# hari-krishnan/openglottal

Measured on AMD Instinct MI355X. Metric: frames/sec 256×256 U-Net-only (frames resident in HBM), higher is better.
Workload: dtype f32; 1 GPU; U-Net-only 256x256 grayscale synthetic video (BASELINE configs[1]; configs[3] with --total-frames 10000), features (32,64,128,256), frames = RandomState(1234+i) BGR -> gray, frame loop u8->/255->UNet->sigmoid->>0.5->area, gray frames resident in HBM, int32 areas left on the device; frames_this_rank=512, frames_per_launch=64, hip_graphs=True, lanes=2

## Files before the change

openglottal_amd/csrc/og_kernels.hpp:

```cpp
#pragma once
#include <hip/hip_runtime.h>
#include <stdint.h>

typedef float f32x16 __attribute__((ext_vector_type(16)));
typedef float f32x4 __attribute__((ext_vector_type(4)));

#define OG_GLOBAL_AS __attribute__((address_space(1)))
#define OG_LDS_AS __attribute__((address_space(3)))

__device__ __forceinline__ void glds16(const float* gsrc, unsigned lds_wave_base) {
    unsigned keep;
    asm volatile(
        "s_mov_b32 %0, m0\n\t"
        "s_mov_b32 m0, %2\n\t"
        "s_nop 0\n\t"
        "global_load_lds_dwordx4 %1, off\n\t"
        "s_mov_b32 m0, %0"
        : "=&s"(keep)
        : "v"(gsrc), "s"(lds_wave_base)
        : "memory");
}
typedef float f32x2 __attribute__((ext_vector_type(2)));
__device__ __forceinline__ f32x2 og_fma2s(f32x2 a, f32x2 b, f32x2 c) { return f32x2{fmaf(a.x, b.x, c.x), fmaf(a.y, b.y, c.y)}; }
__device__ __forceinline__ f32x2 og_fma2(f32x2 a, f32x2 b, f32x2 c) { return __builtin_elementwise_fma(a, b, c); }
// ... 922 lines not shown
    for (int c = c_lo; c < c_hi; ++c) {
#pragma unroll
        for (int t = 0; t < TAPS; ++t) {
            if (VS && ((MODE == 3) ? (t == 0 && c == vnext) : (c * TAPS_ + t == vnext))) {
#pragma unroll
                for (int m = 0; m < MS; ++m) {
#pragma unroll
                    for (int r = 0; r < 16; ++r) {
                        vsum[m][r] += acc[m][r];
                        acc[m][r] = 0.f;
                    }
                }
                ++vp;
                vnext = (vp < vs_n) ? __builtin_amdgcn_readfirstlane((vp * vs_units) / vs_n) : -1;
            }
            if (MODE == 0 && ks_n > 1 && (c * TAPS + t < s_lo || c * TAPS + t >= s_hi)) continue;
            if (MODE == 3) {
                const int par = c / cpc;
                if (((t >> 1) == 0 && (par & 2) == 0) || ((t & 1) == 0 && (par & 1) == 0)) continue;
            }
            const int stg = (NSTG == 3) ? t % 3 : (step & 1), stg_next = (NSTG == 3) ? (t + 1) % 3 : ((step + 1) & 1);
            if (step + 1 < step_end) stage_w(stg_next, step + 1);

            const unsigned wb = (unsigned)stg * WBYTES;
            const int dy = (MODE == 0) ? t / 3 : (MODE == 3) ? (t >> 1) : 0;
            const int dx = (MODE == 0) ? t % 3 : (MODE == 3) ? (t & 1) : 0;
#pragma unroll
            for (int j = 0; j < 4; ++j) {
                const f32x4 bv = og_lds_read16(bbase[j] + wb);
#pragma unroll
                for (int m = 0; m < MS; ++m) {
                    const f32x4 av = og_lds_read16(abase[dx][j ^ ((dy & 1) << 1)] + (unsigned)((dy + 2 * m) * (HW_ * 128)));
                    acc[m] = __builtin_amdgcn_mfma_f32_32x32x2f32(av.x, bv.x, acc[m], 0, 0, 0);
                    acc[m] = __builtin_amdgcn_mfma_f32_32x32x2f32(av.y, bv.y, acc[m], 0, 0, 0);
                    acc[m] = __builtin_amdgcn_mfma_f32_32x32x2f32(av.z, bv.z, acc[m], 0, 0, 0);
                    acc[m] = __builtin_amdgcn_mfma_f32_32x32x2f32(av.w, bv.w, acc[m], 0, 0, 0);
                }
            }
            og_wait_dma();
            __syncthreads();
            ++step;
        }
        if (c + 1 < c_hi) {
            stage_halo(c + 1);
            og_wait_dma();
            __syncthreads();
        }
    }

    if (st != nullptr && tid == 0) st[2] = __builtin_amdgcn_s_memtime();
    if (a.prio_mode == 3) __builtin_amdgcn_s_setprio(3);
    if (VS && vs_n > 1) {
#pragma unroll
        for (int m = 0; m < MS; ++m)
#pragma unroll
            for (int r = 0; r < 16; ++r) acc[m][r] = vsum[m][r] + acc[m][r];
    }
    if (ks_n > 1) {
        float* pw = a.partial + ((long long)item_id * 4 + wave) * (MS * 16 * 64) + lane;
        if (a.tile_counter == nullptr) {
#pragma unroll
            for (int m = 0; m < MS; ++m)
#pragma unroll
                for (int r = 0; r < 16; ++r) pw[(m * 16 + r) * 64] = acc[m][r];
        } else {
#pragma unroll
            for (int m = 0; m < MS; ++m)
#pragma unroll
                for (int r = 0; r < 16; ++r) __hip_atomic_store(pw + (m * 16 + r) * 64, acc[m][r], __ATOMIC_RELAXED, __HIP_MEMORY_SCOPE_AGENT);
        }
        if (a.tile_counter != nullptr) {
            asm volatile("s_waitcnt vmcnt(0)" ::: "memory");
            __syncthreads();
            int* const flag = (int*)smem;
            if (tid == 0) *flag = (atomicAdd(a.tile_counter + tile_id, 1) == ks_n - 1) ? 1 : 0;
            __syncthreads();
            if (*(volatile int*)flag) {
#pragma unroll
                for (int m = 0; m < MS; ++m)
#pragma unroll
                    for (int r = 0; r < 16; ++r) acc[m][r] = 0.f;
                constexpr int PG = (MS == 1) ? 4 : (MS == 2) ? 2 : 1;
                for (int sp_ = 0; sp_ < ks_n; sp_ += PG) {
                    float pv[PG][MS * 16];
#pragma unroll
                    for (int g = 0; g < PG; ++g) {
                        const int sg = (sp_ + g < ks_n) ? sp_ + g : sp_;
                        const float* pr = a.partial + (((long long)tile_id * ks_n + sg) * 4 + wave) * (MS * 16 * 64) + lane;
#pragma unroll
                        for (int k = 0; k < MS * 16; ++k) pv[g][k] = __hip_atomic_load(pr + k * 64, __ATOMIC_RELAXED, __HIP_MEMORY_SCOPE_AGENT);
                    }
#pragma unroll
                    for (int g = 0; g < PG; ++g)
                        if (sp_ + g < ks_n) {
#pragma unroll
                            for (int m = 0; m < MS; ++m)
#pragma unroll
                                for (int r = 0; r < 16; ++r) acc[m][r] += pv[g][m * 16 + r];
                        }
                }
                __syncthreads();
                unsigned char* const scr = smem + wave * 5120;
                if (a.act == 1) conv_epilogue_b<NT, MODE, TH, 1, false>(a, acc, n_tile, b, ty0, tx0, wm, wn, li, lh, esc, esh, scr);
                else if (a.act == 2 && a.res != nullptr) conv_epilogue_b<NT, MODE, TH, 2, true>(a, acc, n_tile, b, ty0, tx0, wm, wn, li, lh, esc, esh, scr);
                else if (a.act == 2) conv_epilogue_b<NT, MODE, TH, 2, false>(a, acc, n_tile, b, ty0, tx0, wm, wn, li, lh, esc, esh, scr);
                else conv_epilogue_b<NT, MODE, TH, 0, false>(a, acc, n_tile, b, ty0, tx0, wm, wn, li, lh, esc, esh, scr);
                if (tid == 0) a.tile_counter[tile_id] = 0;
            }
        }
    } else {
        unsigned char* const scr = smem + wave * 5120;
        if (a.act == 1) conv_epilogue_b<NT, MODE, TH, 1, false>(a, acc, n_tile, b, ty0, tx0, wm, wn, li, lh, esc, esh, scr);
        else if (a.act == 2 && a.res != nullptr) conv_epilogue_b<NT, MODE, TH, 2, true>(a, acc, n_tile, b, ty0, tx0, wm, wn, li, lh, esc, esh, scr);
        else if (a.act == 2) conv_epilogue_b<NT, MODE, TH, 2, false>(a, acc, n_tile, b, ty0, tx0, wm, wn, li, lh, esc, esh, scr);
        else conv_epilogue_b<NT, MODE, TH, 0, false>(a, acc, n_tile, b, ty0, tx0, wm, wn, li, lh, esc, esh, scr);
    }
    if (st != nullptr && tid == 0) {
        asm volatile("s_waitcnt vmcnt(0)" ::: "memory");
        st[3] = __builtin_amdgcn_s_memtime();
    }
}

__device__ __forceinline__ f32x2 og_add2(f32x2 a, f32x2 b) {
    f32x2 r;
    asm volatile("v_pk_add_f32 %0, %1, %2" : "=v"(r) : "v"(a), "v"(b));
    return r;
}
__device__ __forceinline__ f32x2 og_sub2(f32x2 a, f32x2 b) {
    f32x2 r;
    asm volatile("v_pk_add_f32 %0, %1, %2 neg_lo:[0,1] neg_hi:[0,1]" : "=v"(r) : "v"(a), "v"(b));
    return r;
}

template <int NT, int ACT, bool POOL, int HEAD>
__device__ __forceinline__ void wino_tile_end(const ConvArgs& a, const f32x2 (&p)[2][4][4], int n_tile, int b, int ty0, int tx0, int wm, int wn,
                                              int li, int lh, float sc, float sh, unsigned char* scratch) {
    static_assert(NT == 1 || HEAD == 0, "the fused head sits on a 32-column layer");
    constexpr int AREA = 1280;
    const int lane = li + 32 * lh;
    const int cbase = n_tile * 32 * NT + wn * 32;
    const int W = a.W;
    const int ys = ty0 + 8 * wm;
    const int rrow = lane >> 3, rc4 = (lane & 7) * 4;
    const int xl = 2 * (rrow >> 2) + (rrow & 1), yl = (rrow & 3) >> 1;

    const __amdgpu_buffer_rsrc_t out_rs = og_rsrc(a.out + (long long)b * a.out_frame_stride, (unsigned)a.out_frame_stride * 4u);
    unsigned vq[4];
#pragma unroll
    for (int q = 0; q < 4; ++q)
        vq[q] = (tx0 + xl + 4 * q < W) ? (unsigned)(((yl * W + xl + 4 * q) * a.out_pix_stride + rc4) * 4) : OG_OOB;
    unsigned so = (unsigned)(((ys * W + tx0) * a.out_pix_stride + a.out_ch_off + cbase) * 4);
    const unsigned so_step = (unsigned)(2 * W * a.out_pix_stride * 4);

    float* const fw = (float*)scratch + (128 * lh + li);
    const float* const fr = (const float*)scratch + rrow * 32 + rc4;
    __amdgpu_buffer_rsrc_t pool_rs = out_rs;
    unsigned vpool = 0, pso = 0, pso_step = 0;
    if (POOL) {
        pool_rs = og_rsrc(a.pool + (long long)b * a.pool_frame_stride, (unsigned)a.pool_frame_stride * 4u);
        vpool = (tx0 + 2 * rrow < W) ? (unsigned)((rrow * a.pool_pix_stride + rc4) * 4) : OG_OOB;
        pso = (unsigned)((((ys >> 1) * (W >> 1) + (tx0 >> 1)) * a.pool_pix_stride + a.pool_ch_off + cbase) * 4);
        pso_step = (unsigned)((W >> 1) * a.pool_pix_stride * 4);
    }
    f32x4 wv = {0.f, 0.f, 0.f, 0.f};
    int hbx1 = 0, hby1 = 0, hbx2 = 1 << 30, hby2 = 1 << 30, head_cnt = 0;
    const int hk = lane & 7;
    unsigned vh = OG_OOB;
    unsigned hso = 0;
    __amdgpu_buffer_rsrc_t lrs = out_rs, mrs = out_rs;
    if (HEAD) {
        wv = *(const f32x4*)(a.head_w + rc4);
        if (a.head_boxes != nullptr) {
            hbx1 = a.head_boxes[b * 4 + 0];
            hby1 = a.head_boxes[b * 4 + 1];
            hbx2 = a.head_boxes[b * 4 + 2];
            hby2 = a.head_boxes[b * 4 + 3];
            if (hbx1 < 0) { hbx1 = hby1 = hbx2 = hby2 = 0; }
        }
        if (hk < 4 && tx0 + xl + 4 * hk < W) vh = (unsigned)(yl * W + xl + 4 * hk);
        hso = (unsigned)(ys * W + tx0);
        const unsigned long long hfo = (unsigned long long)((long long)b * a.H * W);
        lrs = og_rsrc((const void*)((unsigned long long)a.head_logits + hfo * 4ull), a.head_logits ? (unsigned)(a.H * W) * 4u : 0u);
        mrs = og_rsrc((const void*)((unsigned long long)a.head_mask + hfo), a.head_mask ? (unsigned)(a.H * W) : 0u);
    }

    const f32x2 sc2 = {sc, sc}, sh2 = {sh, sh};
#pragma unroll
    for (int mp = 0; mp < 2; ++mp) {
        f32x2 vmaxs[4];
#pragma unroll
        for (int g = 0; g < 4; ++g) {
#pragma unroll
            for (int rr = 0; rr < 4; ++rr) {
                f32x2 v = og_fma2(p[mp][g][rr], sc2, sh2);
                if (ACT == 1) v = f32x2{fmaxf(v.x, 0.f), fmaxf(v.y, 0.f)};
                fw[(8 * g + rr) * 32] = v.x;
                fw[AREA + (8 * g + rr) * 32] = v.y;
                if (POOL) vmaxs[g] = (rr == 0) ? v : f32x2{fmaxf(vmaxs[g].x, v.x), fmaxf(vmaxs[g].y, v.y)};
            }
        }
        if (POOL) {
#pragma unroll
            for (int g = 0; g < 4; ++g) {
                fw[1024 - 96 * lh + g * 64] = vmaxs[g].x;
                fw[AREA + 1024 - 96 * lh + g * 64] = vmaxs[g].y;
            }
        }
        f32x4 v4[2][4], p4[2];
#pragma unroll
        for (int s = 0; s < 2; ++s) {
#pragma unroll
            for (int q = 0; q < 4; ++q) v4[s][q] = *(const f32x4*)(fr + s * AREA + q * 256);
            if (POOL) p4[s] = *(const f32x4*)(fr + s * AREA + 1024);
        }
#pragma unroll
        for (int s = 0; s < 2; ++s) {
            if (HEAD != 1) {
#pragma unroll
                for (int q = 0; q < 4; ++q) og_buffer_store16(v4[s][q], out_rs, vq[q], so);
                so += so_step;
            }
            if (HEAD) {
                float sd[4];
#pragma unroll
                for (int q = 0; q < 4; ++q) {
                    float sdot = 0.f;
                    sdot = fmaf(v4[s][q].x, wv.x, sdot);
                    sdot = fmaf(v4[s][q].y, wv.y, sdot);
                    sdot = fmaf(v4[s][q].z, wv.z, sdot);
                    sdot = fmaf(v4[s][q].w, wv.w, sdot);
                    sdot += __shfl_xor(sdot, 1);
                    sdot += __shfl_xor(sdot, 2);
                    sdot += __shfl_xor(sdot, 4);
                    sd[q] = sdot;
                }
                float mine = sd[3];
                mine = (hk == 2) ? sd[2] : mine;
                mine = (hk == 1) ? sd[1] : mine;
                mine = (hk == 0) ? sd[0] : mine;
                const float lg = mine + a.head_bias;
                const float prob = 1.0f / (1.0f + expf(-lg));
                const bool on = prob > a.head_thr;
                const int x = tx0 + xl + 4 * hk, y = ys + 2 * (2 * mp + s) + yl;
                const bool counted = on && vh != OG_OOB && x >= hbx1 && x < hbx2 && y >= hby1 && y < hby2;
                head_cnt += __builtin_popcountll(__ballot(counted));
                __builtin_amdgcn_raw_buffer_store_b32(__builtin_bit_cast(unsigned, lg), lrs, (vh == OG_OOB) ? OG_OOB : vh * 4u, hso * 4u, 0);
                __builtin_amdgcn_raw_buffer_store_b8((unsigned char)(on ? 255 : 0), mrs, vh, hso, 0);
                hso += 2u * (unsigned)W;
            }
            if (POOL) {
                og_buffer_store16(p4[s], pool_rs, vpool, pso);
                pso += pso_step;
            }
        }
    }
    if (HEAD && a.head_area != nullptr) {
        if (lane == 0) {
            const int tile = (ty0 / 32) * a.tiles_x + (tx0 >> 4);
            a.head_area[((long long)b * a.tiles_x * a.tiles_y + tile) * 4 + wm] = head_cnt;
        }
    }
}

template <int NT>
__global__ __launch_bounds__(256, 1) void k_conv_wino(ConvArgs a) {
    constexpr int KC = 8 * NT;
    constexpr int PB = KC * 4;
    constexpr int SL = KC / 4;
    constexpr int KS = KC / 8;
    constexpr int TH = 32 / NT;
    constexpr int RP = 18;
    constexpr int RAW_PIX = (TH + 2) * RP;
    constexpr int RAW_BYTES = RAW_PIX * PB;
    constexpr int V_BYTES = 16 * 4096;
    constexpr int UP_BYTES = 32 * NT * PB;
    constexpr int UG_BYTES = 8 * UP_BYTES;
    constexpr int U_IT = UG_BYTES / 4096;
    constexpr int RAW_PIECES = RAW_PIX * SL;
    constexpr int RAW_IT = (RAW_PIECES + 255) / 256;
    constexpr int NST = 8 * KS;

    extern __shared__ __attribute__((aligned(16))) unsigned char smem[];
    const int tid = threadIdx.x;
    const int lane = tid & 63;
    const int wave = __builtin_amdgcn_readfirstlane(tid >> 6);
    const int wn = (NT == 2) ? (wave & 1) : 0, wm = (NT == 2) ? (wave >> 1) : wave;
    const int li = lane & 31, lh = lane >> 5;

    int n_tile, b;
    og_zdecode(a, (int)blockIdx.z, n_tile, b);
    if (b >= a.frames) return;
    const int ty0 = (int)blockIdx.y * TH, tx0 = (int)blockIdx.x * 16;
    unsigned long long* st = nullptr;
    if (a.stamps != nullptr) {
        const unsigned wg = og_wg_index();
        st = a.stamps + 8ull * (wg < 511u ? wg : 511u);
        if (tid == 0) st[0] = __builtin_amdgcn_s_memtime();
    }

    const og_i32x4 in_rsrc = og_make_rsrc(a.in + (long long)b * a.in_frame_stride + a.in_ch_off,
                                          (unsigned)(a.in_frame_stride - a.in_ch_off) * 4u);
    unsigned hoff[RAW_IT];
    {
        constexpr int QY = (256 / SL) / RP, QR = (256 / SL) % RP;
        const int pc = tid % SL;
        int hy = (tid / SL) / RP, r = (tid / SL) - hy * RP;
#pragma unroll
        for (int it = 0; it < RAW_IT; ++it) {
            const int hx = (r >= 9) ? 2 * (r - 9) + 1 : 2 * r;
            const int gy = ty0 + hy - 1, gx = tx0 + hx - 1;
            const bool inb = it * 256 + tid < RAW_PIECES && (unsigned)gy < (unsigned)a.H && (unsigned)gx < (unsigned)a.W;
            hoff[it] = inb ? (unsigned)((gy * a.W + gx) * a.in_pix_stride * 4 + pc * 16) : OG_OOB;
            hy += QY;
            r += QR;
            if (r >= RP) { r -= RP; hy += 1; }
        }
    }
    const unsigned long long last_mask = __builtin_amdgcn_ballot_w64(((RAW_IT - 1) * 256 + tid) < RAW_PIECES);
    const unsigned lds0 = og_lds_addr(smem);
    const int n_ck = a.n_chunks * (32 / KC);
    const og_i32x4 w_rsrc = og_make_rsrc(a.wpk + (long long)n_tile * n_ck * (16 * UP_BYTES / 4), (unsigned)n_ck * (16u * UP_BYTES));
    const unsigned woff = (unsigned)tid * 16u;
    const unsigned ubase = __builtin_amdgcn_readfirstlane(lds0 + RAW_BYTES + V_BYTES + wave * 1024);
    const unsigned hbase = __builtin_amdgcn_readfirstlane(lds0 + wave * 1024);
    unsigned wso = 0, hso = 0;
    auto u_piece = [&](auto pad_, int stage, int i) {
        glds16b_m0<decltype(pad_)::value != 0>(woff, w_rsrc, wso + i * 4096, ubase + stage * UG_BYTES + i * 4096);
    };
    auto raw_piece = [&](auto pad_, int it) {
        if (it < RAW_IT - 1) glds16b_m0<decltype(pad_)::value != 0>(hoff[it], in_rsrc, hso, hbase + it * 4096);
        else glds16b_m0_masked(hoff[it], in_rsrc, hso, hbase + it * 4096, last_mask);
    };
#pragma unroll
    for (int it = 0; it < RAW_IT; ++it) raw_piece(og_const<1>{}, it);
#pragma unroll
    for (int i = 0; i < U_IT; ++i) u_piece(og_const<1>{}, 0, i);
    wso = UG_BYTES;
    hso = PB;
    if (st != nullptr && tid == 0) st[1] = __builtin_amdgcn_s_memtime();

    const int wxa = 2 * (li >> 3) + ((li >> 2) & 1);
    const int nb = wn * 32 + li;
    unsigned abase[KS], bbase[KS];
#pragma unroll
    for (int j = 0; j < KS; ++j) {
        if (NT == 2) {
            abase[j] = lds0 + RAW_BYTES + ((4 * wm + (li & 3)) * 8 + wxa) * 64 + (((2 * j + lh) ^ (li & 3)) << 4);
            bbase[j] = lds0 + RAW_BYTES + V_BYTES + nb * 64 + (((2 * j + lh) ^ ((nb >> 2) & 3)) << 4);
        } else {
            abase[j] = lds0 + RAW_BYTES + (8 * (4 * wm + (wxa >> 1)) + (li & 3) + 4 * (wxa & 1)) * 32 + ((lh ^ ((wxa >> 1) & 1)) << 4);
            bbase[j] = lds0 + RAW_BYTES + V_BYTES + nb * 32 + ((lh ^ ((nb >> 3) & 1)) << 4);
        }
        asm volatile("" : "+v"(abase[j]));
        asm volatile("" : "+v"(bbase[j]));
    }
    const int qc = tid % SL;
    const int wr = (NT == 2) ? (tid >> 5) : 4 * (tid >> 6) + ((tid >> 1) & 3);
    const int wc = (NT == 2) ? ((tid >> 2) & 7) : ((tid >> 3) & 1) + 2 * ((tid >> 4) & 3);
    const int wt = 8 * wr + wc;
    unsigned rbase = lds0 + (unsigned)((2 * wr * RP + wc) * PB + qc * 16);
    unsigned vwbase = (NT == 2) ? lds0 + RAW_BYTES + (unsigned)(wt * 64 + ((qc ^ (wr & 3)) << 4))
                                : lds0 + RAW_BYTES + (unsigned)((8 * (4 * (wr >> 2) + (wc >> 1)) + (wr & 3) + 4 * (wc & 1)) * 32 + ((qc ^ ((wc >> 1) & 1)) << 4));
    asm volatile("" : "+v"(rbase));
    asm volatile("" : "+v"(vwbase));

    const int ecol = n_tile * 32 * NT + wn * 32 + li;
    const float esc = a.scale[ecol], esh = a.shift[ecol];

    f32x16 acc[16];
#pragma unroll
    for (int k = 0; k < 16; ++k) {
#pragma unroll
        for (int r = 0; r < 16; ++r) acc[k][r] = 0.f;
        asm volatile("" : "+a"(acc[k]));
    }

    f32x4 d[16], t[16], tv[16];
    auto raw_read = [&](int n) {
        const int i = n >> 2, j = n & 3;
        d[n] = og_lds_read16(rbase + (unsigned)((i * RP + (j & 1) * 9 + (j >> 1)) * PB));
    };
    auto row_op = [&](int n) {
        const int r = n >> 2, j = n & 3;
        t[n] = (r == 0) ? og_sub4(d[0 + j], d[8 + j]) : (r == 1) ? og_add4(d[4 + j], d[8 + j]) : (r == 2) ? og_sub4(d[8 + j], d[4 + j]) : og_sub4(d[4 + j], d[12 + j]);
    };
    auto col_op = [&](int n) {
        const int i = n >> 2, cc = n & 3;
        tv[n] = (cc == 0) ? og_sub4(t[4 * i + 0], t[4 * i + 2]) : (cc == 1) ? og_add4(t[4 * i + 1], t[4 * i + 2]) : (cc == 2) ? og_sub4(t[4 * i + 2], t[4 * i + 1])
                                                                                                                     : og_sub4(t[4 * i + 1], t[4 * i + 3]);
    };
    auto v_write = [&](int k) { *(OG_LDS_AS f32x4*)(unsigned long long)(vwbase + (unsigned)(k * 4096)) = tv[k]; };
    auto xf_op = [&](int n) {
        if (n < 16) raw_read(n);
        else if (n < 32) row_op(n - 16);
        else if (n < 48) col_op(n - 32);
        else if (n < 56) v_write(n - 48);
    };
    auto xf4 = [&](int n) { xf_op(n); xf_op(n + 1); xf_op(n + 2); xf_op(n + 3); };

    og_wait_dma();
    if (st != nullptr && tid == 0) st[2] = __builtin_amdgcn_s_memtime();
    __syncthreads();
#pragma unroll
    for (int n = 0; n < 48; ++n) xf_op(n);
#pragma unroll
    for (int k = 0; k < 8; ++k) v_write(k);
    __syncthreads();
    if (st != nullptr && tid == 0) st[3] = __builtin_amdgcn_s_memtime();

    auto group = [&](auto g_, auto nxt_) {
        constexpr int g = decltype(g_)::value;
        constexpr bool NXT = decltype(nxt_)::value != 0;
        constexpr bool MORE_U = (g == 0) || NXT;
        f32x4 fa[2], fb[2];
        fa[0] = og_lds_read16(abase[0] + (unsigned)(8 * g * 4096));
        fb[0] = og_lds_read16(bbase[0] + (unsigned)(g * UG_BYTES));
#pragma unroll
        for (int st = 0; st < NST; ++st) {
            const int k = 8 * g + st / KS;
            const f32x4 av = fa[st & 1], bv = fb[st & 1];
            acc[k] = __builtin_amdgcn_mfma_f32_32x32x2f32(av.x, bv.x, acc[k], 0, 0, 0);
            __builtin_amdgcn_sched_barrier(0);
            if (st + 1 < NST) {
                const int kn = (st + 1) / KS, jn = (st + 1) % KS;
                fa[(st + 1) & 1] = og_lds_read16(abase[jn] + (unsigned)((8 * g + kn) * 4096));
                fb[(st + 1) & 1] = og_lds_read16(bbase[jn] + (unsigned)(g * UG_BYTES + kn * UP_BYTES));
            }
            __builtin_amdgcn_sched_barrier(0);
            acc[k] = __builtin_amdgcn_mfma_f32_32x32x2f32(av.y, bv.y, acc[k], 0, 0, 0);
            __builtin_amdgcn_sched_barrier(0);
            if constexpr (g == 0) {
                if (NT == 2) { if (st < 8) v_write(8 + st); }
                else v_write(8 + st);
            } else if constexpr (NXT) {
                if (NT == 2) {
                    if (st < 2) xf4(8 * st);
                    else if (st >= 3 && st < 7) { xf_op(16 + 4 * (st - 3)); xf_op(16 + 4 * (st - 3) + 1); }
                    else if (st >= 7 && st < 11) { xf_op(32 + 4 * (st - 7)); xf_op(32 + 4 * (st - 7) + 1); }
                    else if (st >= 11 && st < 15) xf_op(48 + 2 * (st - 11));
                } else {
                    if (st < 2) xf4(8 * st);
                    else if (st < 4) xf4(16 + 8 * (st - 2));
                    else if (st < 6) xf4(32 + 8 * (st - 4));
                    else { xf_op(48 + 4 * (st - 6)); xf_op(48 + 4 * (st - 6) + 1); }
                }
            }
            __builtin_amdgcn_sched_barrier(0);
            acc[k] = __builtin_amdgcn_mfma_f32_32x32x2f32(av.z, bv.z, acc[k], 0, 0, 0);
            __builtin_amdgcn_sched_barrier(0);
            if constexpr (MORE_U) {
                if (st < U_IT) u_piece(og_const<0>{}, g ^ 1, st);
            }
            if constexpr (g == 1 && NXT) {
                if (NT == 2) {
                    if (st < 2) xf4(8 * st + 4);
                    else if (st >= 3 && st < 7) { xf_op(16 + 4 * (st - 3) + 2); xf_op(16 + 4 * (st - 3) + 3); }
                    else if (st >= 7 && st < 11) { xf_op(32 + 4 * (st - 7) + 2); xf_op(32 + 4 * (st - 7) + 3); }
                    else if (st >= 11 && st < 15) xf_op(48 + 2 * (st - 11) + 1);
                } else {
                    if (st < 2) xf4(8 * st + 4);
                    else if (st < 4) xf4(16 + 8 * (st - 2) + 4);
                    else if (st < 6) xf4(32 + 8 * (st - 4) + 4);
                    else { xf_op(48 + 4 * (st - 6) + 2); xf_op(48 + 4 * (st - 6) + 3); }
                }
            }
            __builtin_amdgcn_sched_barrier(0);
            acc[k] = __builtin_amdgcn_mfma_f32_32x32x2f32(av.w, bv.w, acc[k], 0, 0, 0);
            __builtin_amdgcn_sched_barrier(0);
            if constexpr (g == 0 && NXT) {
                if (st < RAW_IT) raw_piece(og_const<0>{}, st);
            }
            __builtin_amdgcn_sched_barrier(0);
        }
        wso += UG_BYTES;
        if constexpr (g == 0) hso += PB;
        og_wait_dma();
        __syncthreads();
    };
    for (int c = 0; c < n_ck - 1; ++c) {
        group(og_const<0>{}, og_const<1>{});
        group(og_const<1>{}, og_const<1>{});
    }
    group(og_const<0>{}, og_const<0>{});
    group(og_const<1>{}, og_const<0>{});

    if (st != nullptr && tid == 0) st[4] = __builtin_amdgcn_s_memtime();
    f32x2 o[2][4][4];
#pragma unroll
    for (int mp = 0; mp < 2; ++mp) {
#pragma unroll
        for (int g = 0; g < 4; ++g) {
            const int r = 4 * g + 2 * mp;
#pragma unroll
            for (int k = 0; k < 16; ++k) asm volatile("" : "+a"(acc[k]));
            f32x2 tm[2][4];
#pragma unroll
            for (int j = 0; j < 4; ++j) {
                const f32x2 m0 = {acc[0 + j][r], acc[0 + j][r + 1]}, m1 = {acc[4 + j][r], acc[4 + j][r + 1]};
                const f32x2 m2 = {acc[8 + j][r], acc[8 + j][r + 1]}, m3 = {acc[12 + j][r], acc[12 + j][r + 1]};
                tm[0][j] = og_add2(og_add2(m0, m1), m2);
                tm[1][j] = og_sub2(og_sub2(m1, m2), m3);
            }
#pragma unroll
            for (int y = 0; y < 2; ++y) {
                o[mp][g][2 * y + 0] = og_add2(og_add2(tm[y][0], tm[y][1]), tm[y][2]);
                o[mp][g][2 * y + 1] = og_sub2(og_sub2(tm[y][1], tm[y][2]), tm[y][3]);
            }
        }
    }
    if (st != nullptr && tid == 0) st[5] = __builtin_amdgcn_s_memtime();
    unsigned char* const scr = smem + wave * 10240;
    {
        const bool pool = a.pool != nullptr;
        const int head = (NT == 1 && a.head_w != nullptr) ? (a.head_store_act ? 2 : 1) : 0;
        auto end = [&](auto act_, auto pool_, auto head_) {
            wino_tile_end<NT, decltype(act_)::value, decltype(pool_)::value != 0, decltype(head_)::value>(a, o, n_tile, b, ty0, tx0, wm, wn, li, lh, esc, esh, scr);
        };
        auto by_head = [&](auto act_, auto pool_) {
            if constexpr (NT == 1) {
                if (head == 1) end(act_, pool_, og_const<1>{});
                else if (head == 2) end(act_, pool_, og_const<2>{});
                else end(act_, pool_, og_const<0>{});
            } else end(act_, pool_, og_const<0>{});
        };
        auto by_pool = [&](auto act_) {
            if (pool) by_head(act_, og_const<1>{});
            else by_head(act_, og_const<0>{});
        };
        if (a.act == 1) by_pool(og_const<1>{});
        else by_pool(og_const<0>{});
    }
    if (st != nullptr && tid == 0) {
        st[6] = __builtin_amdgcn_s_memtime();
        asm volatile("s_waitcnt vmcnt(0)" ::: "memory");
        st[7] = __builtin_amdgcn_s_memtime();
    }
}

__device__ __forceinline__ void og_store16_dev(float* p, f32x4 v) {
    asm volatile("global_store_dwordx4 %0, %1, off sc1\n\ts_nop 1" : : "v"(p), "v"(v) : "memory");
}
__device__ __forceinline__ f32x4 og_load16_dev(__amdgpu_buffer_rsrc_t rs, unsigned voff, unsigned soff) {
    return __builtin_bit_cast(f32x4, __builtin_amdgcn_raw_buffer_load_b128(rs, voff, soff, 16));
}

template <int NT, int PN>
__global__ __launch_bounds__(256, 1) void k_conv_wino_ps(ConvArgs a) {
    static_assert(PN == 1 || PN == 2 || PN == 4, "a workgroup's positions share one row of the 4x4 position grid");
    constexpr int KC = 8 * NT;
    constexpr int PB = KC * 4;
    constexpr int SL = KC / 4;
    constexpr int KS = KC / 8;
    constexpr int TH = 32 / NT;
    constexpr int RP = 18;
    constexpr int RAW_PIX = (TH + 2) * RP;
    constexpr int RAW_PIECES = RAW_PIX * SL;
    constexpr int RAW_IT = (RAW_PIECES + 255) / 256;
    constexpr int RAW_PAD = RAW_IT * 4096;
    constexpr int UP_BYTES = 32 * NT * PB;
    constexpr int U_STAGE = (PN * UP_BYTES > 4096) ? PN * UP_BYTES : 4096;
    constexpr int U_IT = U_STAGE / 4096;
    constexpr int NDMA = RAW_IT + U_IT;
    constexpr int NPG = 16 / PN;
    constexpr int LA = (PN <= 2) ? 3 : 2;
    constexpr int RS = LA, US = LA + 1;
    constexpr int VB = RS * RAW_PAD;
    constexpr int UB = VB + 2 * PN * 4096;

    extern __shared__ __attribute__((aligned(16))) unsigned char smem[];
    const int tid = threadIdx.x;
    const int lane = tid & 63;
    const int wave = __builtin_amdgcn_readfirstlane(tid >> 6);
    const int wn = (NT == 2) ? (wave & 1) : 0, wm = (NT == 2) ? (wave >> 1) : wave;
    const int li = lane & 31, lh = lane >> 5;

    const int bzf = (int)blockIdx.z;
    const int pg = bzf % NPG, bz = bzf / NPG;
    int n_tile, b;
    og_zdecode(a, bz, n_tile, b);
    if (b >= a.frames) return;
    unsigned long long* const st = a.stamps ? a.stamps + 4ull * (og_wg_index() < 1023u ? og_wg_index() : 1023u) : nullptr;
    if (st != nullptr && tid == 0) st[0] = __builtin_amdgcn_s_memtime();
    const int ty0 = (int)blockIdx.y * TH, tx0 = (int)blockIdx.x * 16;
    const int tile_id = ((b * a.tiles_y + (int)blockIdx.y) * a.tiles_x + (int)blockIdx.x) * a.zdiv + n_tile;
    const int p0 = pg * PN;
    const int pi = p0 >> 2, pc0 = p0 & 3;
    const int ra = (pi == 0) ? 0 : (pi == 2) ? 2 : 1;
    const int rb = (pi == 0) ? 2 : (pi == 1) ? 2 : (pi == 2) ? 1 : 3;
    const bool rplus = pi == 1;

    const og_i32x4 in_rsrc = og_make_rsrc(a.in + (long long)b * a.in_frame_stride + a.in_ch_off,
                                          (unsigned)(a.in_frame_stride - a.in_ch_off) * 4u);
    unsigned hoff[RAW_IT];
    {
        constexpr int QY = (256 / SL) / RP, QR = (256 / SL) % RP;
        const int pc = tid % SL;
        int hy = (tid / SL) / RP, r = (tid / SL) - hy * RP;
#pragma unroll
        for (int it = 0; it < RAW_IT; ++it) {
            const int hx = (r >= 9) ? 2 * (r - 9) + 1 : 2 * r;
            const int gy = ty0 + hy - 1, gx = tx0 + hx - 1;
            const bool inb = it * 256 + tid < RAW_PIECES && (unsigned)gy < (unsigned)a.H && (unsigned)gx < (unsigned)a.W;
            hoff[it] = inb ? (unsigned)((gy * a.W + gx) * a.in_pix_stride * 4 + pc * 16) : OG_OOB;
            hy += QY;
            r += QR;
            if (r >= RP) { r -= RP; hy += 1; }
        }
    }
    const unsigned lds0 = og_lds_addr(smem);
    const int n_ck = a.n_chunks * (32 / KC);
    const og_i32x4 w_rsrc = og_make_rsrc(a.wpk + (long long)n_tile * n_ck * (16 * UP_BYTES / 4), (unsigned)n_ck * (16u * UP_BYTES));
    auto stage = [&](int ck) {
        const unsigned rbase_ = __builtin_amdgcn_readfirstlane(lds0 + (unsigned)((ck % RS) * RAW_PAD) + wave * 1024);
#pragma unroll
        for (int it = 0; it < RAW_IT; ++it) glds16b(hoff[it], in_rsrc, (unsigned)ck * PB, rbase_ + it * 4096);
        const unsigned ubase_ = __builtin_amdgcn_readfirstlane(lds0 + UB + (unsigned)((ck % US) * U_STAGE) + wave * 1024);
#pragma unroll
        for (int i = 0; i < U_IT; ++i)
            glds16b((unsigned)tid * 16u, w_rsrc, (unsigned)((ck * 16 + p0) * UP_BYTES + i * 4096), ubase_ + i * 4096);
    };
#pragma unroll
    for (int i = 0; i < LA; ++i)
        if (i < n_ck) stage(i);

    const int wxa = 2 * (li >> 3) + ((li >> 2) & 1);
    const int nb = wn * 32 + li;
    unsigned abase[KS], bbase[KS];
#pragma unroll
    for (int j = 0; j < KS; ++j) {
        if (NT == 2) {
            abase[j] = lds0 + VB + ((4 * wm + (li & 3)) * 8 + wxa) * 64 + (((2 * j + lh) ^ (li & 3)) << 4);
            bbase[j] = lds0 + UB + nb * 64 + (((2 * j + lh) ^ ((nb >> 2) & 3)) << 4);
        } else {
            abase[j] = lds0 + VB + (8 * (4 * wm + (wxa >> 1)) + (li & 3) + 4 * (wxa & 1)) * 32 + ((lh ^ ((wxa >> 1) & 1)) << 4);
            bbase[j] = lds0 + UB + nb * 32 + ((lh ^ ((nb >> 3) & 1)) << 4);
        }
    }
    const int qc = tid % SL;
    const int wr = (NT == 2) ? (tid >> 5) : 4 * (tid >> 6) + ((tid >> 1) & 3);
    const int wc = (NT == 2) ? ((tid >> 2) & 7) : ((tid >> 3) & 1) + 2 * ((tid >> 4) & 3);
    const int wt = 8 * wr + wc;
    const unsigned rbase = lds0 + (unsigned)((2 * wr * RP + wc) * PB + qc * 16);
    const unsigned vwbase = (NT == 2) ? lds0 + VB + (unsigned)(wt * 64 + ((qc ^ (wr & 3)) << 4))
                                      : lds0 + VB + (unsigned)((8 * (4 * (wr >> 2) + (wc >> 1)) + (wr & 3) + 4 * (wc & 1)) * 32 + ((qc ^ ((wc >> 1) & 1)) << 4));

    int issued = ((n_ck < LA) ? n_ck : LA) - 1;
    auto wait_landed = [&](int ck) {
        const int newer = issued - ck;
        if (LA >= 3 && newer >= 2) asm volatile("s_waitcnt vmcnt(%0)" ::"n"(2 * NDMA) : "memory");
        else if (newer == 1) asm volatile("s_waitcnt vmcnt(%0)" ::"n"(NDMA) : "memory");
        else og_wait_dma();
    };
    const float rsgn = rplus ? 1.0f : -1.0f;
    constexpr int NCOL = (PN == 1) ? 2 : (PN == 2) ? 3 : 4;
    int colj[NCOL];
    if (PN == 1) {
        colj[0] = (pc0 == 0) ? 0 : (pc0 == 2) ? 2 : 1;
        colj[1] = (pc0 == 0) ? 2 : (pc0 == 1) ? 2 : (pc0 == 2) ? 1 : 3;
    } else if (PN == 2) {
        colj[0] = pc0 ? 1 : 0;
        colj[1] = pc0 ? 2 : 1;
        colj[NCOL - 1] = pc0 ? 3 : 2;
    } else {
#pragma unroll
        for (int j = 0; j < NCOL; ++j) colj[j] = j;
    }
    f32x4 xa[NCOL], xb[NCOL];
    auto tr_read = [&](int ck) {
        const unsigned rb_ = rbase + (unsigned)((ck % RS) * RAW_PAD);
#pragma unroll
        for (int n = 0; n < NCOL; ++n) {
            const int j = colj[n];
            xa[n] = og_lds_read16(rb_ + (unsigned)((ra * RP + (j & 1) * 9 + (j >> 1)) * PB));
            xb[n] = og_lds_read16(rb_ + (unsigned)((rb * RP + (j & 1) * 9 + (j >> 1)) * PB));
        }
    };
    auto fma4 = [](float sgn, f32x4 b_, f32x4 a_) {
        const f32x2 s2 = {sgn, sgn};
        f32x2 lo, hi;
        asm("v_pk_fma_f32 %0, %1, %2, %3" : "=v"(lo) : "v"(s2), "v"(f32x2{b_.x, b_.y}), "v"(f32x2{a_.x, a_.y}));
        asm("v_pk_fma_f32 %0, %1, %2, %3" : "=v"(hi) : "v"(s2), "v"(f32x2{b_.z, b_.w}), "v"(f32x2{a_.z, a_.w}));
        return f32x4{lo.x, lo.y, hi.x, hi.y};
    };
    auto tr_write = [&](int ck) {
        f32x4 t[NCOL];
#pragma unroll
        for (int n = 0; n < NCOL; ++n) t[n] = fma4(rsgn, xb[n], xa[n]);
#pragma unroll
        for (int k = 0; k < PN; ++k) {
            f32x4 v;
            if (PN == 1) v = fma4((pc0 == 1) ? 1.0f : -1.0f, t[1], t[0]);
            else if (PN == 2) {
                if (k == 0) v = pc0 ? fma4(-1.0f, t[0], t[1]) : fma4(-1.0f, t[2], t[0]);
                else v = pc0 ? fma4(-1.0f, t[2], t[0]) : fma4(1.0f, t[2], t[1]);
            } else v = (k == 0) ? og_sub4(t[0], t[2]) : (k == 1) ? og_add4(t[1], t[2]) : (k == 2) ? og_sub4(t[2], t[1]) : og_sub4(t[1], t[3]);
            *(OG_LDS_AS f32x4*)(unsigned long long)(vwbase + (unsigned)(((ck & 1) * PN + k) * 4096)) = v;
        }
    };

    f32x16 acc[PN];
#pragma unroll
    for (int k = 0; k < PN; ++k)
#pragma unroll
        for (int r = 0; r < 16; ++r) acc[k][r] = 0.f;

    wait_landed(0);
    __syncthreads();
    tr_read(0);
    tr_write(0);
    if (n_ck > 1) wait_landed(1);
    if (st != nullptr && tid == 0) st[1] = __builtin_amdgcn_s_memtime();

    for (int c = 0; c < n_ck; ++c) {
        __syncthreads();
        if (c + LA < n_ck) {
            stage(c + LA);
            issued = c + LA;
        }
        if (c + 1 < n_ck) tr_read(c + 1);
        const unsigned vo = (unsigned)((c & 1) * PN * 4096), uo = (unsigned)((c % US) * U_STAGE);
        f32x4 fa[2], fb[2];
        fa[0] = og_lds_read16(abase[0] + vo);
        fb[0] = og_lds_read16(bbase[0] + uo);
#pragma unroll
        for (int s_ = 0; s_ < PN * KS; ++s_) {
            const int k = s_ / KS;
            if (s_ + 1 < PN * KS) {
                const int kn = (s_ + 1) / KS, jn = (s_ + 1) % KS;
                fa[(s_ + 1) & 1] = og_lds_read16(abase[jn] + vo + (unsigned)(kn * 4096));
                fb[(s_ + 1) & 1] = og_lds_read16(bbase[jn] + uo + (unsigned)(kn * UP_BYTES));
            }
            const f32x4 av = fa[s_ & 1], bv = fb[s_ & 1];
            __builtin_amdgcn_sched_barrier(0);
            acc[k] = __builtin_amdgcn_mfma_f32_32x32x2f32(av.x, bv.x, acc[k], 0, 0, 0);
            acc[k] = __builtin_amdgcn_mfma_f32_32x32x2f32(av.y, bv.y, acc[k], 0, 0, 0);
            acc[k] = __builtin_amdgcn_mfma_f32_32x32x2f32(av.z, bv.z, acc[k], 0, 0, 0);
            acc[k] = __builtin_amdgcn_mfma_f32_32x32x2f32(av.w, bv.w, acc[k], 0, 0, 0);
            __builtin_amdgcn_sched_barrier(0);
        }
        if (c + 1 < n_ck) tr_write(c + 1);
        if (c + 2 < n_ck) wait_landed(c + 2);
    }

    if (st != nullptr && tid == 0) st[2] = __builtin_amdgcn_s_memtime();
    float* const part = a.partial + (long long)tile_id * (16 * 4 * 1024) + wave * 1024 + lane * 4;
#pragma unroll
    for (int k = 0; k < PN; ++k)
#pragma unroll
        for (int q = 0; q < 4; ++q)
            og_store16_dev(part + (p0 + k) * 4096 + q * 256, f32x4{acc[k][4 * q], acc[k][4 * q + 1], acc[k][4 * q + 2], acc[k][4 * q + 3]});
    asm volatile("s_waitcnt vmcnt(0)" ::: "memory");
    __syncthreads();
    int* const flag = (int*)smem;
    if (tid == 0) *flag = (atomicAdd(a.tile_counter + tile_id, 1) == NPG - 1) ? 1 : 0;
    __syncthreads();
    if (*(volatile int*)flag == 0) {
        if (st != nullptr && tid == 0) st[3] = __builtin_amdgcn_s_memtime();
        return;
    }
    __syncthreads();

    const int ecol = n_tile * 32 * NT + wn * 32 + li;
    const float esc = a.scale[ecol], esh = a.shift[ecol];
    const __amdgpu_buffer_rsrc_t part_rs = og_rsrc(a.partial + (long long)tile_id * (16 * 4 * 1024), 16u * 4u * 1024u * 4u);
    const unsigned part_voff = (unsigned)((wave * 1024 + lane * 4) * 4);
    f32x16 o[4];
    {
        f32x4 mm[4][16];
#pragma unroll
        for (int q = 0; q < 4; ++q)
#pragma unroll
            for (int k = 0; k < 16; ++k) mm[q][k] = og_load16_dev(part_rs, part_voff, (unsigned)((k * 4096 + q * 256) * 4));
#pragma unroll
        for (int q = 0; q < 4; ++q) {
            const f32x4* const m = mm[q];
#pragma unroll
            for (int e = 0; e < 4; ++e) {
                float tm[2][4];
#pragma unroll
                for (int j = 0; j < 4; ++j) {
                    tm[0][j] = m[0 + j][e] + m[4 + j][e] + m[8 + j][e];
                    tm[1][j] = m[4 + j][e] - m[8 + j][e] - m[12 + j][e];
                }
#pragma unroll
                for (int y = 0; y < 2; ++y) {
                    o[e][4 * q + 2 * y + 0] = tm[y][0] + tm[y][1] + tm[y][2];
                    o[e][4 * q + 2 * y + 1] = tm[y][1] - tm[y][2] - tm[y][3];
                }
            }
        }
// ... 3136 lines not shown
```

Baseline: 9770 frames/s.

## Overlap weight prefetch with first input transform in Winograd conv prologue

Simplifies the per-thread halo offset computation, using a cheaper strength-reduced path with bounds checks only for edge tiles. The raw input DMA is now issued before the weight DMA, so the kernel waits only for the raw pieces (vmcnt(U_IT)) before starting the input transform, while the weight loads are still in flight. The transform is reordered into two halves with sched barriers and the full DMA wait is moved after it. The scale/shift loads are also moved later, and an alignment nop is added before the epilogue. Main risk is a small gain or a register/scheduling regression in the prologue.

```diff
diff --git a/openglottal_amd/csrc/og_kernels.hpp b/openglottal_amd/csrc/og_kernels.hpp
--- a/openglottal_amd/csrc/og_kernels.hpp
+++ b/openglottal_amd/csrc/og_kernels.hpp
@@ -1248,37 +1248,42 @@
                                           (unsigned)(a.in_frame_stride - a.in_ch_off) * 4u);
     unsigned hoff[RAW_IT];
     {
-        constexpr int QY = (256 / SL) / RP, QR = (256 / SL) % RP;
-        const int pc = tid % SL;
-        int hy = (tid / SL) / RP, r = (tid / SL) - hy * RP;
-#pragma unroll
-        for (int it = 0; it < RAW_IT; ++it) {
-            const int hx = (r >= 9) ? 2 * (r - 9) + 1 : 2 * r;
-            const int gy = ty0 + hy - 1, gx = tx0 + hx - 1;
-            const bool inb = it * 256 + tid < RAW_PIECES && (unsigned)gy < (unsigned)a.H && (unsigned)gx < (unsigned)a.W;
-            hoff[it] = inb ? (unsigned)((gy * a.W + gx) * a.in_pix_stride * 4 + pc * 16) : OG_OOB;
-            hy += QY;
-            r += QR;
-            if (r >= RP) { r -= RP; hy += 1; }
-        }
-    }
-    const unsigned long long last_mask = __builtin_amdgcn_ballot_w64(((RAW_IT - 1) * 256 + tid) < RAW_PIECES);
+        const unsigned col_b = (unsigned)a.in_pix_stride * 4u, row_b = (unsigned)a.W * col_b;
+        const unsigned corner = (unsigned)(ty0 - 1) * row_b + (unsigned)(tx0 - 1) * col_b + (unsigned)(tid % SL) * 16u;
+        auto offsets = [&](auto edge_) {
+            unsigned p = (unsigned)tid / SL;
+#pragma unroll
+            for (int it = 0; it < RAW_IT; ++it) {
+                const unsigned hy = p / RP, r = p - hy * RP;
+                const unsigned hx = (r >= 9) ? 2 * r - 17 : 2 * r;
+                unsigned off = corner + hy * row_b + __umul24(hx, col_b);
+                if (decltype(edge_)::value != 0) off = ((unsigned)(tx0 - 1) + hx < (unsigned)a.W) ? off : OG_OOB;
+                hoff[it] = off;
+                p += 256 / SL;
+            }
+        };
+        if (tx0 == 0 || tx0 + 16 >= a.W) offsets(og_const<1>{});
+        else offsets(og_const<0>{});
+    }
     const unsigned lds0 = og_lds_addr(smem);
     const int n_ck = a.n_chunks * (32 / KC);
-    const og_i32x4 w_rsrc = og_make_rsrc(a.wpk + (long long)n_tile * n_ck * (16 * UP_BYTES / 4), (unsigned)n_ck * (16u * UP_BYTES));
-    const unsigned woff = (unsigned)tid * 16u;
-    const unsigned ubase = __builtin_amdgcn_readfirstlane(lds0 + RAW_BYTES + V_BYTES + wave * 1024);
     const unsigned hbase = __builtin_amdgcn_readfirstlane(lds0 + wave * 1024);
     unsigned wso = 0, hso = 0;
-    auto u_piece = [&](auto pad_, int stage, int i) {
-        glds16b_m0<decltype(pad_)::value != 0>(woff, w_rsrc, wso + i * 4096, ubase + stage * UG_BYTES + i * 4096);
-    };
+    unsigned long long last_mask = 0;
     auto raw_piece = [&](auto pad_, int it) {
         if (it < RAW_IT - 1) glds16b_m0<decltype(pad_)::value != 0>(hoff[it], in_rsrc, hso, hbase + it * 4096);
         else glds16b_m0_masked(hoff[it], in_rsrc, hso, hbase + it * 4096, last_mask);
     };
 #pragma unroll
-    for (int it = 0; it < RAW_IT; ++it) raw_piece(og_const<1>{}, it);
+    for (int it = 0; it < RAW_IT - 1; ++it) raw_piece(og_const<1>{}, it);
+    last_mask = __builtin_amdgcn_ballot_w64(((RAW_IT - 1) * 256 + tid) < RAW_PIECES);
+    raw_piece(og_const<1>{}, RAW_IT - 1);
+    const og_i32x4 w_rsrc = og_make_rsrc(a.wpk + (long long)n_tile * n_ck * (16 * UP_BYTES / 4), (unsigned)n_ck * (16u * UP_BYTES));
+    const unsigned woff = (unsigned)tid * 16u;
+    const unsigned ubase = __builtin_amdgcn_readfirstlane(lds0 + RAW_BYTES + V_BYTES + wave * 1024);
+    auto u_piece = [&](auto pad_, int stage, int i) {
+        glds16b_m0<decltype(pad_)::value != 0>(woff, w_rsrc, wso + i * 4096, ubase + stage * UG_BYTES + i * 4096);
+    };
 #pragma unroll
     for (int i = 0; i < U_IT; ++i) u_piece(og_const<1>{}, 0, i);
     wso = UG_BYTES;
@@ -1309,9 +1314,6 @@
                                 : lds0 + RAW_BYTES + (unsigned)((8 * (4 * (wr >> 2) + (wc >> 1)) + (wr & 3) + 4 * (wc & 1)) * 32 + ((qc ^ ((wc >> 1) & 1)) << 4));
     asm volatile("" : "+v"(rbase));
     asm volatile("" : "+v"(vwbase));
-
-    const int ecol = n_tile * 32 * NT + wn * 32 + li;
-    const float esc = a.scale[ecol], esh = a.shift[ecol];
 
     f32x16 acc[16];
 #pragma unroll
@@ -1344,13 +1346,31 @@
     };
     auto xf4 = [&](int n) { xf_op(n); xf_op(n + 1); xf_op(n + 2); xf_op(n + 3); };
 
-    og_wait_dma();
+    asm volatile("s_waitcnt vmcnt(%0)" : : "n"(U_IT) : "memory");
+    const int ecol = n_tile * 32 * NT + wn * 32 + li;
+    const float esc = a.scale[ecol], esh = a.shift[ecol];
     if (st != nullptr && tid == 0) st[2] = __builtin_amdgcn_s_memtime();
     __syncthreads();
 #pragma unroll
-    for (int n = 0; n < 48; ++n) xf_op(n);
+    for (int n = 0; n < 8; ++n) raw_read(8 * (n & 1) + (n >> 1));
+#pragma unroll
+    for (int n = 4; n < 8; ++n) raw_read(n);
+#pragma unroll
+    for (int n = 12; n < 16; ++n) raw_read(n);
+    __builtin_amdgcn_sched_barrier(0);
+#pragma unroll
+    for (int n = 0; n < 8; ++n) row_op(n);
+#pragma unroll
+    for (int n = 0; n < 8; ++n) col_op(n);
 #pragma unroll
     for (int k = 0; k < 8; ++k) v_write(k);
+    __builtin_amdgcn_sched_barrier(0);
+#pragma unroll
+    for (int n = 8; n < 16; ++n) row_op(n);
+#pragma unroll
+    for (int n = 8; n < 16; ++n) col_op(n);
+    __builtin_amdgcn_sched_barrier(0);
+    og_wait_dma();
     __syncthreads();
     if (st != nullptr && tid == 0) st[3] = __builtin_amdgcn_s_memtime();
 
@@ -1432,6 +1452,7 @@
 
     if (st != nullptr && tid == 0) st[4] = __builtin_amdgcn_s_memtime();
     f32x2 o[2][4][4];
+    asm volatile(".p2align 3\n\ts_nop 0");
 #pragma unroll
     for (int mp = 0; mp < 2; ++mp) {
 #pragma unroll
```

After: 9858 frames/s, median of 6. No clear change (+0.9%).
